# xeTaiz/vit-tf

Hardware: AMD Instinct MI355X
Metric: slices/sec (ViT-S/8, 512^3 vol: feature volume + 16-query similarity) (higher is better)
Workload: dtype fp16; 1 GPU; 512^3 CT-like synthetic volume (seed 0), ViT-S/8, fos 64: 1536 slices of 512x512 (N=4097) per step + 16-query similarity -> the metric's configuration (BASELINE configs[2]); engine_batch=512, weights=seeded synthetic vits8 (seed 0), parallelism=single GPU

## Files before the change

vit-tf_amd/csrc/engine.hip:

```cpp
#include "vittf_internal.h"

#include <stdlib.h>
#include <vector>

namespace {
struct ProfRec { hipEvent_t a, b; int cls; };
unsigned g_prof_mask = 0;
std::vector<ProfRec> g_prof_recs;
std::vector<hipEvent_t> g_prof_pool;

hipEvent_t prof_event() {
  if (!g_prof_pool.empty()) { hipEvent_t e = g_prof_pool.back(); g_prof_pool.pop_back(); return e; }
  hipEvent_t e;
  (void)hipEventCreate(&e);
  return e;
}

struct WsLayout {
  size_t x, h, qkv, o, fp8, fp8_bytes, tile_ctr, total;
};

WsLayout ws_layout(int d, int64_t rows, size_t fp8_bytes = 0) {
  const int64_t rp = (rows + 127) / 128 * 128;
  WsLayout l;
// ... 85 lines not shown
  if (((uintptr_t)ws & 255) != 0) return VITTF_ERR_INVALID_ARG;
  char* base = (char*)ws;
  float* X = (float*)(base + lay.x);
  void* H = base + lay.h;
  void* QKV = base + lay.qkv;
  void* O = base + lay.o;
  void* G = QKV;

  int rc;
  { ProfScope ps(VITTF_KERNEL_PATCH_EMBED, stream); rc = vittf_patch_embed_reg(cfg, w, pos, view, slice0, batch, reg_rows, n_reg, X, stream); }
  if (rc) return rc;
  const size_t esz = 2;
  const bool res_ln = !(cfg->flags & VITTF_CFG_SEPARATE_LN) && (d == 384 || d == 768);
  const int pre = (cfg->flags & VITTF_CFG_UNSCALED_Q) ? 0 : 1;
  const bool fp8_rows = !(cfg->flags & VITTF_CFG_FP8_HEAD_SCALES) && cfg->attention_fp8 && pre && d >= 768 && d % 256 == 0;
  const bool tail = d == 384 && w->tail_packed && res_ln;
  const bool qkv_as = d == 384 && w->qkv_packed && !cfg->attention_fp8;
  for (int l = 0; l < L; ++l) {
    const char* qkv_w = (const char*)w->qkv_w + (size_t)l * 3 * d * d * esz;
    if (res_ln ? l == 0 : true) {
      ProfScope ps(VITTF_KERNEL_LAYERNORM, stream);
      rc = vittf_layernorm(X, w->ln1_g + (size_t)l * d, w->ln1_b + (size_t)l * d, H, rows, d, cfg->ln_eps, dt, stream);
      if (rc) return rc;
    }
    if (l == L - 1 && (part_mask & 7)) {
      ProfScope ps(VITTF_KERNEL_GEMM, stream);
      rc = vittf_gemm_kfeat_parts_reg(H, qkv_w, w->qkv_b + (size_t)l * 3 * d, rows, d, d, tokens, n_reg, part_mask & 7, q_out,
                                      k_out, v_out, dt, stream);
      if (rc || !want_t) return rc;
    }
    const float* next_g = l == L - 1 ? norm_g : w->ln1_g + (size_t)(l + 1) * d;
    const float* next_b = l == L - 1 ? norm_b : w->ln1_b + (size_t)(l + 1) * d;
    { ProfScope ps(VITTF_KERNEL_GEMM_QKV, stream);
      if (fp8_rows)
        rc = vittf_gemm_qkv_fp8(H, qkv_w, w->qkv_b + (size_t)l * 3 * d, QKV, rows, 3 * d, d, tokens, cfg->heads, dt,
                                base + lay.fp8, lay.fp8_bytes, stream);
      else if (qkv_as)
        rc = vittf_gemm_as(H, (const char*)w->qkv_packed + (size_t)l * 3 * d * d * esz, w->qkv_b + (size_t)l * 3 * d, QKV, rows, 3 * d, d,
                           pre ? VITTF_EPI_BIAS_QKV : VITTF_EPI_BIAS, dt, base + lay.tile_ctr, stream);
      else
        rc = vittf_gemm(H, qkv_w, w->qkv_b + (size_t)l * 3 * d, QKV, rows, 3 * d, d,
                        pre ? VITTF_EPI_BIAS_QKV : VITTF_EPI_BIAS, 0, dt, stream);
      if (!rc && rope) rc = vittf_rope_qk(QKV, rows, tokens, 1 + n_reg, cfg->heads, rope, dt, stream); }
    if (rc) return rc;
    { ProfScope ps(VITTF_KERNEL_ATTENTION, stream);
      if (fp8_rows)
        rc = vittf_attention_fp8_rows(QKV, O, batch, tokens, cfg->heads, dt, base + lay.fp8, lay.fp8_bytes, stream);
      else if (cfg->attention_fp8 && pre)
        rc = vittf_attention_fp8(QKV, O, batch, tokens, cfg->heads, dt, base + lay.fp8, lay.fp8_bytes, stream);
      else
        rc = vittf_attention(QKV, O, batch, tokens, cfg->heads, dt, pre, stream); }
    if (rc) return rc;
    if (tail) {
      ProfScope ps(VITTF_KERNEL_MLP, stream);
      rc = vittf_block_tail(O, (const char*)w->tail_packed + (size_t)l * VITTF_TAIL_STEPS * 12288 * esz, w->proj_b + (size_t)l * d,
                            w->ln2_g + (size_t)l * d, w->ln2_b + (size_t)l * d, w->fc1_b + (size_t)l * 4 * d,
                            w->fc2_b + (size_t)l * d, X, rows, d, dt, next_g, next_b, cfg->ln_eps, H, base + lay.tile_ctr,
                            stream);
      if (rc) return rc;
      continue;
    }
    { ProfScope ps(VITTF_KERNEL_GEMM_PROJ, stream);
      if (res_ln)
        rc = vittf_gemm_residual_ln(O, (const char*)w->proj_w + (size_t)l * d * d * esz, w->proj_b + (size_t)l * d, X, rows, d,
                                    d, dt, w->ln2_g + (size_t)l * d, w->ln2_b + (size_t)l * d, cfg->ln_eps, H, stream);
      else
        rc = vittf_gemm(O, (const char*)w->proj_w + (size_t)l * d * d * esz, w->proj_b + (size_t)l * d, X, rows, d, d,
                        VITTF_EPI_BIAS_RESIDUAL, 0, dt, stream); }
    if (rc) return rc;
    if (!res_ln) {
      ProfScope ps(VITTF_KERNEL_LAYERNORM, stream);
      rc = vittf_layernorm(X, w->ln2_g + (size_t)l * d, w->ln2_b + (size_t)l * d, H, rows, d, cfg->ln_eps, dt, stream);
      if (rc) return rc;
    }
    { ProfScope ps(VITTF_KERNEL_GEMM_FC1, stream);
      rc = vittf_gemm(H, (const char*)w->fc1_w + (size_t)l * 4 * d * d * esz, w->fc1_b + (size_t)l * 4 * d, G, rows,
                      4 * d, d, VITTF_EPI_BIAS_GELU, 0, dt, stream); }
    if (rc) return rc;
    { ProfScope ps(VITTF_KERNEL_GEMM_FC2, stream);
      if (res_ln)
        rc = vittf_gemm_residual_ln(G, (const char*)w->fc2_w + (size_t)l * 4 * d * d * esz, w->fc2_b + (size_t)l * d, X, rows,
                                    d, 4 * d, dt, next_g, next_b, cfg->ln_eps, H, stream);
      else
        rc = vittf_gemm(G, (const char*)w->fc2_w + (size_t)l * 4 * d * d * esz, w->fc2_b + (size_t)l * d, X, rows, d,
                        4 * d, VITTF_EPI_BIAS_RESIDUAL, 0, dt, stream); }
    if (rc) return rc;
  }
  ProfScope ps(VITTF_KERNEL_LAYERNORM, stream);
  return vittf_token_features(X, norm_g, norm_b, t_out, batch, tokens, 1 + n_reg, d, cfg->ln_eps, stream);
}

extern "C" int vittf_vit_qkv_features_rope(const vittf_vit_config* cfg, const vittf_vit_weights* w, const vittf_pos_embed* pos,
                                           const vittf_slice_view* view, int32_t slice0, int32_t batch, int32_t part_mask,
                                           const float* reg_rows, int32_t n_reg, const vittf_rope_table* rope, uint16_t* q_out,
                                           uint16_t* k_out, uint16_t* v_out, void* ws, size_t ws_bytes, void* stream) {
  if (part_mask <= 0 || part_mask > 7) return VITTF_ERR_INVALID_ARG;
  return vittf_vit_features(cfg, w, pos, view, slice0, batch, part_mask, reg_rows, n_reg, rope, nullptr, nullptr, q_out, k_out,
                            v_out, nullptr, ws, ws_bytes, stream);
}

extern "C" int vittf_vit_qkv_features_reg(const vittf_vit_config* cfg, const vittf_vit_weights* w, const vittf_pos_embed* pos,
                                          const vittf_slice_view* view, int32_t slice0, int32_t batch, int32_t part_mask,
                                          const float* reg_rows, int32_t n_reg, uint16_t* q_out, uint16_t* k_out,
                                          uint16_t* v_out, void* ws, size_t ws_bytes, void* stream) {
  return vittf_vit_qkv_features_rope(cfg, w, pos, view, slice0, batch, part_mask, reg_rows, n_reg, nullptr, q_out, k_out, v_out, ws,
                                     ws_bytes, stream);
}

extern "C" int vittf_vit_qkv_features(const vittf_vit_config* cfg, const vittf_vit_weights* w, const vittf_pos_embed* pos,
                                      const vittf_slice_view* view, int32_t slice0, int32_t batch, int32_t part_mask,
                                      uint16_t* q_out, uint16_t* k_out, uint16_t* v_out, void* ws, size_t ws_bytes,
// ... 43 lines not shown
```

vit-tf_amd/csrc/tail_fx.hip:

```cpp
#include "vittf_common.h"

#include <type_traits>
#include <utility>

namespace {

constexpr int D = 384, HID = 4 * D, UNITS = HID / 32;
constexpr int SB = 24576, HB = SB / 2;
constexpr int PSTEPS = D / 32;
constexpr int LAG = 4;
constexpr int MSTEPS = 2 * UNITS + LAG;
constexpr int NSEQ = PSTEPS + MSTEPS;
constexpr int NSLOT = 4, AHEAD = NSLOT - 1;
constexpr int PIECES = SB / 1024 / 4;
constexpr int WAIT0 = (AHEAD - 2) * PIECES;
constexpr int NF = 4;
constexpr int PB_OFF = NSLOT * SB;
constexpr int PBH = 4608, PB = 2 * PBH;
constexpr int STG_ROW = 144;
constexpr int AF_SLOT = 1056, AF_H = 528;
constexpr int CONST_OFF = PB_OFF + 4 * PB;
constexpr int C_B1 = 0, C_B2 = HID, C_G1 = HID + D, C_E1 = HID + 2 * D,
              C_BP = HID + 3 * D, C_G2 = HID + 4 * D, C_E2 = HID + 5 * D,
              C_N = HID + 6 * D;
constexpr int NEXT_OFF = CONST_OFF + C_N * 4;
constexpr int LDS_BYTES = NEXT_OFF + 16;
static_assert(LDS_BYTES <= 160 * 1024, "LDS");
static_assert(AHEAD >= 3, "ring depth");
static_assert(32 * STG_ROW <= PBH && 4 * AF_SLOT <= PBH, "pair buffer");

typedef __attribute__((ext_vector_type(4))) unsigned u32x4_t;
typedef __attribute__((ext_vector_type(2))) unsigned u32x2_t;
typedef __attribute__((address_space(3))) const s16x8_t* lds_frag_ptr;
typedef __attribute__((address_space(3))) const f32x4_t* lds_f4_ptr;
typedef __attribute__((address_space(3))) f32x4_t* lds_w4_ptr;
typedef __attribute__((address_space(3))) u32x4_t* lds_wu4_ptr;
typedef __attribute__((address_space(3))) u32x2_t* lds_w2_ptr;
typedef __attribute__((address_space(3))) volatile unsigned* lds_u32_ptr;

struct Ring {
  i32x4_t rsrc;
  unsigned dma_dst;
  int src0;
  int g;
  int slot;
};

__device__ __forceinline__ s16x8_t ld_frag(const unsigned (&base)[4], int f) {
  return *(lds_frag_ptr)(base[f & 3] + (f >> 2) * 4096);
}

__device__ __forceinline__ void lds_dma16_keep(i32x4_t rsrc, unsigned lds_addr, int voff, int soff) {
  asm volatile("s_mov_b32 m0, %0\n\ts_nop 0\n\tbuffer_load_dwordx4 %1, %2, %3 offen lds"
               :: "s"(lds_addr), "v"(voff), "s"(rsrc), "s"(soff) : "memory");
}

struct Gelu3 { float x, p; };
__device__ __forceinline__ void gelu_a(Gelu3& s, float x) {
  s.x = x;
  asm volatile("" : "+v"(s.x));
  s.p = fmaf(-0.000524238159f, fabsf(s.x), 0.00741911121f);
  s.p = fmaf(s.p, fabsf(s.x), -0.0526018888f);
  s.p = fmaf(s.p, fabsf(s.x), -0.459225923f);
  asm volatile("" : "+v"(s.x), "+v"(s.p));
}
__device__ __forceinline__ void gelu_b(Gelu3& s) {
  s.p = fmaf(s.p, fabsf(s.x), -1.15109742f);
  s.p = __builtin_amdgcn_exp2f(fmaf(s.p, fabsf(s.x), -1.0f));
  asm volatile("" : "+v"(s.p));
}
__device__ __forceinline__ float gelu_c(const Gelu3& s) {
  float v = fmaf(-fabsf(s.x), s.p, fmaxf(s.x, 0.f));
  asm volatile("" : "+v"(v));
  return v;
}

template <int WAITN, bool LGKM = false>
__device__ __forceinline__ void x_wait() {
  static_assert(WAITN <= 63, "vmcnt");
  if constexpr (WAITN < 0) {
    if constexpr (LGKM) asm volatile("s_waitcnt lgkmcnt(0)\n\ts_barrier" ::: "memory");
    else asm volatile("s_barrier" ::: "memory");
// ... 57 lines not shown
      const int r = 8 * KH + 2 * (j / 3);
      if (j % 3 == 0) {
        gelu_a(s0, gprev[r]); gelu_a(s1, gprev[r + 1]);
      } else if (j % 3 == 1) {
        gelu_b(s0); gelu_b(s1);
      } else {
        const float v0 = gelu_c(s0), v1 = gelu_c(s1);
        pk[j / 3] = pack2_h16<DT>(v0, v1);
      }
    }
    __builtin_amdgcn_sched_barrier(0);
  }
  ring_advance(st);
}

template <int DT, int OH, bool LAST>
__device__ __forceinline__ void x_step(Ring& st, unsigned (&base)[4], s16x8_t (&wf)[NF], f32x16_t (&xacc)[D / 32],
                                       s16x8_t (&gf)[2], unsigned gf_addr) {
  x_wait<WAIT0>();
  const int g_next = ring_next(st), slot_free = ring_free(st);
  if constexpr (OH == 0) {
    gf[0] = *(lds_frag_ptr)(gf_addr);
    gf[1] = *(lds_frag_ptr)(gf_addr + 1024);
  }
#pragma unroll
  for (int j = 0; j < 12; ++j) {
    xacc[6 * OH + (j >> 1)] = mfma32<DT>(wf[j % NF], gf[j & 1], xacc[6 * OH + (j >> 1)]);
    ring_gap<LAST, true>(st, base, wf, j, g_next, slot_free);
    __builtin_amdgcn_sched_barrier(0);
  }
  ring_advance(st);
}

template <int DT, int WAITN, bool FIRST, bool LAST>
__device__ __forceinline__ void p_step(Ring& st, unsigned (&base)[4], s16x8_t (&wf)[NF], f32x16_t (&xacc)[D / 32],
                                       const s16x8_t (&acur)[2], s16x8_t (&anext)[2], unsigned anext_addr0, unsigned anext_addr1) {
  if constexpr (!FIRST) x_wait<WAITN>();
  const int g_next = ring_next(st), slot_free = ring_free(st);
  if constexpr (!LAST) {
    anext[0] = *(lds_frag_ptr)(anext_addr0);
    anext[1] = *(lds_frag_ptr)(anext_addr1);
  }
#pragma unroll
  for (int j = 0; j < 24; ++j) {
    xacc[j % 12] = mfma32<DT>(wf[j % NF], acur[j / 12], xacc[j % 12]);
    ring_gap<LAST, true, 24>(st, base, wf, j, g_next, slot_free);
    __builtin_amdgcn_sched_barrier(0);
  }
  ring_advance(st);
}

__device__ __forceinline__ constexpr int af_off(int s) { return (((s >> 2) & 1) ? 0 : PBH) + (s & 3) * AF_SLOT; }

struct Ctx {
  const unsigned short* abuf; const unsigned short* wpk; float* x; unsigned short* hout; unsigned* tile_ctr;
  int64_t rows; float ln_eps; int ntiles; int tile; unsigned lds0;
};
__device__ __forceinline__ unsigned uni(unsigned v) { return __builtin_amdgcn_readfirstlane(v); }
template <typename T> __device__ __forceinline__ T* uni_ptr(T* p) {
  const uint64_t v = reinterpret_cast<uint64_t>(p);
  return reinterpret_cast<T*>(((uint64_t)uni((unsigned)(v >> 32)) << 32) | uni((unsigned)v));
}
#define FX_ROLE_ENV                                                                                                       \
  const unsigned short* const abuf = uni_ptr(c.abuf);                                                                     \
  float* const x = uni_ptr(c.x);                                                                                          \
  unsigned short* const hout = uni_ptr(c.hout);                                                                           \
  unsigned* const tile_ctr = uni_ptr(c.tile_ctr);                                                                         \
  const int64_t rows = (int64_t)(((uint64_t)uni((unsigned)((uint64_t)c.rows >> 32)) << 32) | uni((unsigned)c.rows));     \
  const float ln_eps = __uint_as_float(uni(__float_as_uint(c.ln_eps)));                                                   \
  const int ntiles = (int)uni((unsigned)c.ntiles);                                                                        \
  int tile = (int)uni((unsigned)c.tile);                                                                                  \
  const unsigned lds0 = uni(c.lds0);                                                                                      \
  const int tid = threadIdx.x;                                                                                            \
  const int lane = tid & 63, wave = __builtin_amdgcn_readfirstlane(tid >> 6);                                             \
  const int rb = wave & 3;                                                                                                \
  const int h = lane >> 5, l31 = lane & 31;                                                                               \
  unsigned cl = lds0 + CONST_OFF + 16 * h;                                                                                \
  asm volatile("" : "+v"(cl));                                                                                            \
  auto cst4 = [&](int i) { return *(lds_f4_ptr)(cl + 4 * i); };             \
  const unsigned nxt = lds0 + NEXT_OFF;                                                                                   \
  Ring st;                                                                                                                \
  st.rsrc = lds_dma_rsrc(uni_ptr(c.wpk), (unsigned)(NSEQ * SB));                                                          \
  st.src0 = rb * (PIECES * 1024);                                                                                         \
  st.dma_dst = lds0;                                                                                                      \
  st.g = 0;                                                                                                               \
  st.slot = 0;                                                                                                            \
  const int aoff0 = tile_off(l31, h);                                                                                     \
  const unsigned pbuf = lds0 + PB_OFF + rb * PB;                           \
   \
  auto tile_rsrc = [&](const void* p, int64_t tile, int row_bytes) {                                                      \
    const int64_t first = tile * 128, left = rows - first;                                                                \
    const int nrows = tile < 0 || left <= 0 || !p ? 0 : left < 128 ? (int)left : 128;                                     \
    return __builtin_amdgcn_make_buffer_rsrc(const_cast<char*>(reinterpret_cast<const char*>(p)) + (nrows ? first : 0) * row_bytes, 0, \
                                             nrows * row_bytes, 0x00020000);                                              \
  };                                                                                                                      \
  (void)abuf; (void)x; (void)hout; (void)tile_ctr; (void)ln_eps; (void)ntiles; (void)l31; (void)aoff0; (void)nxt; (void)cst4; (void)tile_rsrc

template <int DT>
__device__ __attribute__((noinline)) void run_f(Ctx c) {
  FX_ROLE_ENV;
  asm volatile("s_setprio 3");
  unsigned pbl = pbuf + lane * 16;
  asm volatile("" : "+v"(pbl));
  u32x4_t fb[48];
  const int q8 = lane >> 3, c8 = lane & 7;
  __amdgpu_buffer_rsrc_t ra, rx;
  const int ao = (rb * 32 + q8) * (D * 2) + c8 * 16, xo = (rb * 32 + q8) * (D * 4) + c8 * 16;
  auto load_a = [&](int cg) {
#pragma unroll
    for (int i = 0; i < 4; ++i) fb[4 * cg + i] = __builtin_amdgcn_raw_buffer_load_b128(ra, ao + cg * 128, i * 8 * (D * 2), 0);
  };
  auto load_chunk = [&](int c) {
    const int r0 = c < 6 ? 24 + 4 * c : 4 * (c - 6);
#pragma unroll
    for (int i = 0; i < 4; ++i) fb[r0 + i] = __builtin_amdgcn_raw_buffer_load_b128(rx, xo + c * 128, i * 8 * (D * 4), 0);
  };
  const unsigned af_wr = pbuf + (c8 >> 1) * AF_SLOT + (c8 & 1) * AF_H + q8 * 16;
  auto put_a = [&](int cg) {
#pragma unroll
    for (int i = 0; i < 4; ++i) *(lds_wu4_ptr)(af_wr + af_off(4 * cg) + i * 128) = fb[4 * cg + i];
  };
  const unsigned ch_wr = pbuf + q8 * STG_ROW + c8 * 16;
  auto put_chunk = [&](int c) {
    const int r0 = c < 6 ? 24 + 4 * c : 4 * (c - 6);
#pragma unroll
    for (int i = 0; i < 4; ++i) *(lds_wu4_ptr)(ch_wr + (c & 1) * PBH + i * 8 * STG_ROW) = fb[r0 + i];
  };
  auto fetch_rows = [&](int t) {
    ra = tile_rsrc(abuf, t, D * 2);
    rx = tile_rsrc(x, t, D * 4);
#pragma unroll
    for (int cg = 0; cg < 6; ++cg) load_a(cg);
#pragma unroll
    for (int c = 0; c < 6; ++c) load_chunk(c);
    put_a(0);
  };
  fetch_rows(tile);
  asm volatile("s_waitcnt vmcnt(0)" ::: "memory");
  __syncthreads();
  while (true) {
    unsigned next_v = 0;
    if (tid == 256) next_v = atomicAdd(tile_ctr, 1u);
    unsigned base[4];
    s16x8_t hf[D / 16];
    s16x8_t wf[NF];
    f32x16_t bias_c;
    auto load_bias = [&](int at) {
#pragma unroll
      for (int q = 0; q < 4; ++q) {
// ... 35 lines not shown
    for (int f = 0; f < NF; ++f) wf[f] = ld_frag(base, f);
#pragma unroll
    for (int j = 0; j < 12; ++j) {
      ga = mfma32<DT>(wf[j % NF], hf[j], j == 0 ? bias_c : ga);
      ring_gap<false, false>(st, base, wf, j, 0, 0);
      __builtin_amdgcn_sched_barrier(0);
    }
    ring_advance(st);
    f_step<DT, 1, false, false, false>(st, base, wf, hf, ga, bias_c, gb, pk1);
    for (int u = 1; u < UNITS - 1; u += 2) {
      load_bias(C_B1 + 32 * u);
      f_step<DT, 0, true, false, true>(st, base, wf, hf, gb, bias_c, ga, pk0);
      f_step<DT, 1, true, false, false>(st, base, wf, hf, gb, bias_c, ga, pk1);
      put_gf(0);
      load_bias(C_B1 + 32 * (u + 1));
      f_step<DT, 0, true, false, true>(st, base, wf, hf, ga, bias_c, gb, pk0);
      f_step<DT, 1, true, false, false>(st, base, wf, hf, ga, bias_c, gb, pk1);
      put_gf(1);
    }
    load_bias(C_B1 + 32 * (UNITS - 1));
    f_step<DT, 0, true, false, true>(st, base, wf, hf, gb, bias_c, ga, pk0);
    f_step<DT, 1, true, true, false>(st, base, wf, hf, gb, bias_c, ga, pk1);
    put_gf(0);
    sync_wait<true>();
    ring_advance(st);
#pragma unroll
    for (int r = 0; r < 16; r += 2) {
      const float v0 = gelu_poly(gb[r]), v1 = gelu_poly(gb[r + 1]);
      const unsigned w = pack2_h16<DT>(v0, v1);
      if (r < 8) pk0[r >> 1] = w; else pk1[(r - 8) >> 1] = w;
    }
    put_gf(1);
    sync_wait<true>(); ring_advance(st);
    sync_wait(); ring_advance(st);
    sync_wait(); ring_advance(st);
    if (tid == 256) *(lds_u32_ptr)nxt = next_v;
    asm volatile("s_waitcnt vmcnt(0) lgkmcnt(0)\n\ts_barrier" ::: "memory");
    const int next = __builtin_amdgcn_readfirstlane((int)*(lds_u32_ptr)nxt);
    if (next >= ntiles) break;
    tile = next;
    fetch_rows(tile);
  }
}

template <int DT>
__device__ __attribute__((noinline)) void run_x(Ctx c) {
  FX_ROLE_ENV;
  unsigned base[4];
  asm volatile("s_waitcnt vmcnt(0)" ::: "memory");
  __syncthreads();
  s16x8_t wf[NF];
  f32x16_t xacc[D / 32];
  while (true) {
    int ln = lane;
    asm volatile("" : "+v"(ln));
    {
#pragma unroll
      for (int ot = 0; ot < D / 32; ++ot)
#pragma unroll
        for (int q = 0; q < 4; ++q) {
          const f32x4_t bv = cst4(C_BP + 32 * ot + 8 * q);
          xacc[ot][4 * q + 0] = bv[0]; xacc[ot][4 * q + 1] = bv[1]; xacc[ot][4 * q + 2] = bv[2]; xacc[ot][4 * q + 3] = bv[3];
        }
#pragma unroll
      for (int i = 0; i < 4; ++i) base[i] = lds0 + st.slot * SB + (aoff0 ^ (32 * i));
      const unsigned af_rd = pbuf + (ln >> 5) * AF_H + (ln & 31) * 16;
      s16x8_t aa[2], ab[2];
      x_wait<-1, true>();
#pragma unroll
      for (int f = 0; f < NF; ++f) wf[f] = ld_frag(base, f);
      aa[0] = *(lds_frag_ptr)(af_rd + af_off(0));
      aa[1] = *(lds_frag_ptr)(af_rd + af_off(1));
      p_step<DT, -1, true, false>(st, base, wf, xacc, aa, ab, af_rd + af_off(2), af_rd + af_off(3));
      p_step<DT, -1, false, false>(st, base, wf, xacc, ab, aa, af_rd + af_off(4), af_rd + af_off(5));
#pragma unroll
      for (int p = 2; p < PSTEPS - 2; p += 2) {
        p_step<DT, WAIT0, false, false>(st, base, wf, xacc, aa, ab, af_rd + af_off(2 * p + 2), af_rd + af_off(2 * p + 3));
        p_step<DT, WAIT0, false, false>(st, base, wf, xacc, ab, aa, af_rd + af_off(2 * p + 4), af_rd + af_off(2 * p + 5));
      }
      p_step<DT, WAIT0, false, false>(st, base, wf, xacc, aa, ab, af_rd + af_off(2 * PSTEPS - 2), af_rd + af_off(2 * PSTEPS - 1));
      p_step<DT, WAIT0, false, true>(st, base, wf, xacc, ab, aa, 0, 0);
      const unsigned ch_rd = pbuf + (ln & 31) * STG_ROW + 16 * (ln >> 5);
#pragma unroll
      for (int r = 0; r < 12; ++r) {
        sync_wait<true>();
        f32x4_t xv[4];
#pragma unroll
        for (int g = 0; g < 4; ++g) xv[g] = *(lds_f4_ptr)(ch_rd + (r & 1) * PBH + 32 * g);
#pragma unroll
        for (int g = 0; g < 4; ++g)
#pragma unroll
          for (int e = 0; e < 4; ++e) xacc[r][4 * g + e] += xv[g][e];
      }
      float s = 0.f;
#pragma unroll
      for (int ot = 0; ot < D / 32; ++ot) {
#pragma unroll
        for (int g = 0; g < 4; ++g) s += (xacc[ot][4 * g + 0] + xacc[ot][4 * g + 1]) + (xacc[ot][4 * g + 2] + xacc[ot][4 * g + 3]);
        __builtin_amdgcn_sched_barrier(0);
      }
      {
        const auto sw = __builtin_amdgcn_permlane32_swap(__float_as_uint(s), __float_as_uint(s), false, false);
        s = __uint_as_float(sw[0]) + __uint_as_float(sw[1]);
      }
      const float mean = s / (float)D;
      float q = 0.f;
#pragma unroll
      for (int ot = 0; ot < D / 32; ++ot) {
#pragma unroll
        for (int r = 0; r < 16; ++r) { const float dv = xacc[ot][r] - mean; q += dv * dv; }
        __builtin_amdgcn_sched_barrier(0);
      }
      {
        const auto sw = __builtin_amdgcn_permlane32_swap(__float_as_uint(q), __float_as_uint(q), false, false);
        q = __uint_as_float(sw[0]) + __uint_as_float(sw[1]);
      }
      const float rstd = 1.0f / sqrtf(q / (float)D + ln_eps);
      float mean_p = mean;
      asm volatile("" : "+v"(mean_p));
      const unsigned hw_ = pbuf + ln * 16;
      f32x4_t gq[2][4], bq[2][4];
#pragma unroll
      for (int g = 0; g < 4; ++g) { gq[0][g] = cst4(C_G2 + 8 * g); bq[0][g] = cst4(C_E2 + 8 * g); }
#pragma unroll
      for (int ot = 0; ot < D / 32; ++ot) {
        if (ot + 1 < D / 32) {
#pragma unroll
          for (int g = 0; g < 4; ++g) { gq[(ot + 1) & 1][g] = cst4(C_G2 + 32 * (ot + 1) + 8 * g); bq[(ot + 1) & 1][g] = cst4(C_E2 + 32 * (ot + 1) + 8 * g); }
        }
#pragma unroll
        for (int k2 = 0; k2 < 2; ++k2) {
          u32x4_t pk;
#pragma unroll
          for (int g2_ = 0; g2_ < 2; ++g2_) {
            const int g = 2 * k2 + g2_;
            const f32x4_t gg = gq[ot & 1][g], bb = bq[ot & 1][g];
            pk[2 * g2_ + 0] = pack2_h16<DT>((xacc[ot][4 * g + 0] - mean_p) * rstd * gg[0] + bb[0], (xacc[ot][4 * g + 1] - mean_p) * rstd * gg[1] + bb[1]);
            pk[2 * g2_ + 1] = pack2_h16<DT>((xacc[ot][4 * g + 2] - mean_p) * rstd * gg[2] + bb[2], (xacc[ot][4 * g + 3] - mean_p) * rstd * gg[3] + bb[3]);
          }
          *(lds_wu4_ptr)(hw_ + (ot & 1) * PBH + k2 * 1024) = pk;
        }
        sync_wait<true>();
      }
    }
    s16x8_t gf[2];
    x_idle_step<WAIT0>(st); x_idle_step<WAIT0>(st); x_idle_step<WAIT0>(st);
    x_wait<WAIT0>();
    {
      const int g_next = ring_next(st), slot_free = ring_free(st);
#pragma unroll
      for (int i = 0; i < PIECES; ++i) ring_piece(st, i, g_next, slot_free);
      ring_advance(st);
#pragma unroll
      for (int i = 0; i < 4; ++i) base[i] = lds0 + st.slot * SB + HB + (aoff0 ^ (32 * i));
#pragma unroll
      for (int f = 0; f < NF; ++f) wf[f] = ld_frag(base, f);
    }
    const unsigned gfa = pbuf + ln * 16;
    for (int u = 0; u < UNITS - 2; u += 2) {
      x_step<DT, 0, false>(st, base, wf, xacc, gf, gfa);
      x_step<DT, 1, false>(st, base, wf, xacc, gf, gfa);
      x_step<DT, 0, false>(st, base, wf, xacc, gf, gfa + PBH);
      x_step<DT, 1, false>(st, base, wf, xacc, gf, gfa + PBH);
    }
    x_step<DT, 0, false>(st, base, wf, xacc, gf, gfa);
    x_step<DT, 1, false>(st, base, wf, xacc, gf, gfa);
    x_step<DT, 0, false>(st, base, wf, xacc, gf, gfa + PBH);
    x_step<DT, 1, true>(st, base, wf, xacc, gf, gfa + PBH);
    asm volatile("s_waitcnt vmcnt(0) lgkmcnt(0)\n\ts_barrier" ::: "memory");
    const int next = __builtin_amdgcn_readfirstlane((int)*(lds_u32_ptr)nxt);
    {
      const auto rxo = tile_rsrc(x, tile, D * 4);
      const auto rho = tile_rsrc(hout, tile, D * 2);
      int le = lane;
      asm volatile("" : "+v"(le));
      const unsigned stg_wr_e = pbuf + (le & 31) * STG_ROW + 16 * (le >> 5);
      const unsigned stg_wh = pbuf + (le & 31) * STG_ROW + 8 * (le >> 5);
      const unsigned stg_rd_e = pbuf + (le >> 3) * STG_ROW + (le & 7) * 16;
      const int xo_e = (rb * 32 + (le >> 3)) * (D * 4) + (le & 7) * 16;
      const int ho = (rb * 32 + (le >> 3)) * (D * 2) + (le & 7) * 16;
      float s = 0.f;
      {
        f32x4_t bvq[2][4];
#pragma unroll
        for (int g = 0; g < 4; ++g) bvq[0][g] = cst4(C_B2 + 8 * g);
#pragma unroll
        for (int ot = 0; ot < D / 32; ++ot) {
#pragma unroll
          for (int g = 0; g < 4; ++g) {
            const f32x4_t bv = bvq[ot & 1][g];
            f32x4_t v;
            v[0] = xacc[ot][4 * g + 0] + bv[0]; v[1] = xacc[ot][4 * g + 1] + bv[1];
            v[2] = xacc[ot][4 * g + 2] + bv[2]; v[3] = xacc[ot][4 * g + 3] + bv[3];
#pragma unroll
            for (int e = 0; e < 4; ++e) xacc[ot][4 * g + e] = v[e];
            *(lds_w4_ptr)(stg_wr_e + 32 * g) = v;
            s += (v[0] + v[1]) + (v[2] + v[3]);
          }
          __builtin_amdgcn_sched_barrier(0);
          f32x4_t rbk[4];
#pragma unroll
          for (int i = 0; i < 4; ++i) rbk[i] = *(lds_f4_ptr)(stg_rd_e + i * 8 * STG_ROW);
          if (ot + 1 < D / 32) {
#pragma unroll
            for (int g = 0; g < 4; ++g) bvq[(ot + 1) & 1][g] = cst4(C_B2 + 32 * (ot + 1) + 8 * g);
          }
          __builtin_amdgcn_sched_barrier(0);
#pragma unroll
          for (int i = 0; i < 4; ++i)
            __builtin_amdgcn_raw_buffer_store_b128(__builtin_bit_cast(u32x4_t, rbk[i]), rxo, xo_e + ot * 128, i * 8 * (D * 4), 0);
          __builtin_amdgcn_sched_barrier(0);
        }
      }
      if (hout) {
        {
          const auto sw = __builtin_amdgcn_permlane32_swap(__float_as_uint(s), __float_as_uint(s), false, false);
          s = __uint_as_float(sw[0]) + __uint_as_float(sw[1]);
        }
        const float mean = s / (float)D;
        float q = 0.f;
#pragma unroll
        for (int ot = 0; ot < D / 32; ++ot) {
#pragma unroll
          for (int r = 0; r < 16; ++r) { const float dv = xacc[ot][r] - mean; q += dv * dv; }
          __builtin_amdgcn_sched_barrier(0);
        }
        {
          const auto sw = __builtin_amdgcn_permlane32_swap(__float_as_uint(q), __float_as_uint(q), false, false);
          q = __uint_as_float(sw[0]) + __uint_as_float(sw[1]);
        }
        const float rstd = 1.0f / sqrtf(q / (float)D + ln_eps);
        float mean_p = mean;
        asm volatile("" : "+v"(mean_p));
        f32x4_t gq1[2][4], bq1[2][4];
#pragma unroll
        for (int g = 0; g < 4; ++g) { gq1[0][g] = cst4(C_G1 + 8 * g); bq1[0][g] = cst4(C_E1 + 8 * g); }
#pragma unroll
        for (int ot = 0; ot < D / 32; ++ot) {
          const int op = ot >> 1, o2 = ot & 1;
#pragma unroll
          for (int g = 0; g < 4; ++g) {
            const f32x4_t gg = gq1[ot & 1][g], bb = bq1[ot & 1][g];
            u32x2_t pk;
            pk[0] = pack2_h16<DT>((xacc[ot][4 * g + 0] - mean_p) * rstd * gg[0] + bb[0], (xacc[ot][4 * g + 1] - mean_p) * rstd * gg[1] + bb[1]);
            pk[1] = pack2_h16<DT>((xacc[ot][4 * g + 2] - mean_p) * rstd * gg[2] + bb[2], (xacc[ot][4 * g + 3] - mean_p) * rstd * gg[3] + bb[3]);
            *(lds_w2_ptr)(stg_wh + 64 * o2 + 16 * g) = pk;
          }
          __builtin_amdgcn_sched_barrier(0);
          [[maybe_unused]] f32x4_t rbk[4];
          if (o2) {
#pragma unroll
            for (int i = 0; i < 4; ++i) rbk[i] = *(lds_f4_ptr)(stg_rd_e + i * 8 * STG_ROW);
          }
          if (ot + 1 < D / 32) {
#pragma unroll
            for (int g = 0; g < 4; ++g) { gq1[(ot + 1) & 1][g] = cst4(C_G1 + 32 * (ot + 1) + 8 * g); bq1[(ot + 1) & 1][g] = cst4(C_E1 + 32 * (ot + 1) + 8 * g); }
          }
          __builtin_amdgcn_sched_barrier(0);
          if (o2) {
#pragma unroll
            for (int i = 0; i < 4; ++i)
              __builtin_amdgcn_raw_buffer_store_b128(__builtin_bit_cast(u32x4_t, rbk[i]), rho, ho + op * 128, i * 8 * (D * 2), 0);
            __builtin_amdgcn_sched_barrier(0);
          }
        }
      }
    }
    if (next >= ntiles) break;
    tile = next;
  }
}

template <int DT>
__global__ __launch_bounds__(512, 1) void tail_fx_kernel(const unsigned short* __restrict__ abuf, const unsigned short* __restrict__ wpk,
                                                         const float* __restrict__ bp, const float* __restrict__ g2, const float* __restrict__ e2,
                                                         const float* __restrict__ b1, const float* __restrict__ b2,
                                                         float* __restrict__ x, int64_t rows, const float* __restrict__ ln_g,
                                                         const float* __restrict__ ln_b, float ln_eps,
                                                         unsigned short* __restrict__ hout, int ntiles,
                                                         unsigned* __restrict__ tile_ctr) {
  __shared__ __attribute__((aligned(16))) char smem[LDS_BYTES];
  const int tid = threadIdx.x;
  const int lane = tid & 63, wave = __builtin_amdgcn_readfirstlane(tid >> 6);
  float* const cst = reinterpret_cast<float*>(smem + CONST_OFF);
  for (int i = tid; i < C_N; i += 512) {
    float v;
    if (i < C_B2) v = b1[i];
    else if (i < C_G1) v = b2[i - C_B2];
    else if (i < C_E1) v = ln_g ? ln_g[i - C_G1] : 1.f;
    else if (i < C_BP) v = ln_b ? ln_b[i - C_E1] : 0.f;
    else if (i < C_G2) v = bp[i - C_BP];
    else if (i < C_E2) v = g2[i - C_G2];
    else v = e2[i - C_E2];
    cst[i] = v;
  }
  const unsigned lds0 = (unsigned)(size_t)LDS_PTR(smem);
  const unsigned nxt = lds0 + NEXT_OFF;
  if (tid == 0) *(lds_u32_ptr)nxt = atomicAdd(tile_ctr, 1u);
  __syncthreads();
  const int tile = __builtin_amdgcn_readfirstlane((int)*(lds_u32_ptr)nxt);
  if (tile >= ntiles) return;
  if (wave < 4) {
    const i32x4_t rsrc = lds_dma_rsrc(wpk, (unsigned)(NSEQ * SB));
#pragma unroll
    for (int u = 0; u < AHEAD; ++u)
#pragma unroll
      for (int i = 0; i < PIECES; ++i)
        lds_dma16(rsrc, lds0 + wave * (PIECES * 1024) + u * SB + i * 1024, lane * 16, u * SB + wave * (PIECES * 1024) + i * 1024);
  }
  const Ctx c = {abuf, wpk, x, hout, tile_ctr, rows, ln_eps, ntiles, tile, lds0};
  if (wave >= 4) run_f<DT>(c);
  else run_x<DT>(c);
  asm volatile("s_waitcnt vmcnt(0)" ::: "memory");
}

}

extern "C" size_t vittf_block_tail_workspace_bytes(void) { return sizeof(unsigned); }

extern "C" int vittf_block_tail(const void* attn_out, const void* w_packed, const float* proj_b, const float* ln2_g,
                                const float* ln2_b, const float* b1, const float* b2, float* x, int64_t rows, int32_t d,
                                int32_t dtype, const float* ln_g, const float* ln_b, float ln_eps, void* h_out, void* tile_counter,
                                void* stream) {
  if (!attn_out || !w_packed || !proj_b || !ln2_g || !ln2_b || !b1 || !b2 || !x || rows <= 0) return VITTF_ERR_INVALID_ARG;
  if (d != D) return VITTF_ERR_INVALID_ARG;
  if ((ln_g || ln_b || h_out) && !(ln_g && ln_b && h_out)) return VITTF_ERR_INVALID_ARG;
  const int64_t tiles = (rows + 127) / 128;
  if (tiles > 0x7fffffff) return VITTF_ERR_INVALID_ARG;
  if ((((uintptr_t)attn_out | (uintptr_t)w_packed | (uintptr_t)x | (uintptr_t)h_out) & 15) != 0) return VITTF_ERR_INVALID_ARG;
  if (!tile_counter || ((uintptr_t)tile_counter & 3) != 0) return VITTF_ERR_INVALID_ARG;
  const int cus = vittf_current_cus();
  if (cus <= 0) return VITTF_ERR_NO_DEVICE;
  const unsigned grid = (unsigned)(tiles < cus ? tiles : cus);
  hipStream_t st = (hipStream_t)stream;
  unsigned* ctr = (unsigned*)tile_counter;
  if (hipMemsetAsync(ctr, 0, sizeof(unsigned), st) != hipSuccess) return VITTF_ERR_LAUNCH;
#define FX_LAUNCH(DTV)                                                                                               \
  hipLaunchKernelGGL((tail_fx_kernel<DTV>), dim3(grid), dim3(512), 0, st, (const unsigned short*)attn_out,           \
                     (const unsigned short*)w_packed, proj_b, ln2_g, ln2_b, b1, b2, x, rows, ln_g, ln_b, ln_eps,     \
                     (unsigned short*)h_out, (int)tiles, ctr)
  if (dtype == VITTF_BF16) FX_LAUNCH(VITTF_BF16);
  else if (dtype == VITTF_FP16) FX_LAUNCH(VITTF_FP16);
  else return VITTF_ERR_INVALID_ARG;
#undef FX_LAUNCH
  vittf_note_kernel(VITTF_KERNEL_MLP, "tail_fx_kernel");
  return vittf_check_launch();
}
```

vit-tf_amd/csrc/vittf_internal.h:

```cpp
#pragma once
#include "vittf_common.h"

static inline size_t align256(size_t x) { return (x + 255) & ~(size_t)255; }

static inline int64_t vittf_kfeat_out_bytes(int64_t rows, int32_t d, int32_t tokens, int32_t drop) {
  return (rows - rows / tokens * drop) * (int64_t)d * 2;
}

bool vittf_gemm_rows_covers(int32_t n, int32_t k, int64_t rows);
int vittf_gemm_rows(const void* a, const void* w, const float* bias, float* x, int64_t rows, int32_t n, int32_t k,
                    int32_t dtype, const float* ln_g, const float* ln_b, float ln_eps, void* h, hipStream_t st);

bool vittf_gemm_pp_covers(int32_t k, int32_t columns, const void* a, const void* w);
bool vittf_gemm_pp_covers_out(const void* out, int64_t kfeat_bytes);
int vittf_gemm_pp(const void* a, const void* w, const float* bias, void* out, int64_t rows, int32_t n, int32_t k,
                  int32_t epilogue, int32_t tokens, int32_t dtype, hipStream_t st);
int vittf_gemm_pp_kfeat_parts(const void* a, const void* w, const float* bias, int64_t rows, int32_t d, int32_t k,
                              int32_t tokens, int32_t n_reg, int32_t part_mask, void* const outs[3], int32_t dtype,
                              hipStream_t st, int32_t* taken);

void vittf_fp8_ws_pointers(void* ws, int32_t batch, int32_t tokens, int32_t heads, unsigned** amax, unsigned char** q8,
                           unsigned char** k8, unsigned char** qs, unsigned char** ks, int32_t* np);

int vittf_attention_pp64(const void* qkv, void* out, int32_t batch, int32_t tokens, int32_t heads, int32_t dtype,
                         hipStream_t st);

size_t vittf_sim_mfma_workspace_bytes(int32_t classes, int32_t annotations);
bool vittf_sim_mfma_applies(int32_t f, int32_t classes, int32_t total_a, const void* ws, size_t ws_bytes, const void* feat,
                            int64_t nvox);
int vittf_sim_mfma_maps(const unsigned short* feat, int32_t f, int64_t nvox, const float* qf, const int32_t* class_start_host,
                        int32_t classes, const float* voxel_norm, float* sim, unsigned* maxbits, void* ws, size_t ws_bytes,
                        hipStream_t st);
```

Baseline: 2282 slices/s.

## Skip residual store in penultimate tail and double-buffer epilogue LDS staging

Adds a store_x flag to the fused block-tail kernel so the penultimate layer, when only key features are wanted, skips writing the fp32 residual stream back to global memory. The epilogue staging now alternates between the pair buffer and an idle ring slot, so writes for the next column block can proceed before the previous block's read-back and global store finish, and H stores are deferred by one iteration. Lane indices are recomputed via mbcnt to cut live registers. This relies on the last ring slot being unused at drain time; if the final X is needed elsewhere, skipping the store could break correctness.

```diff
diff --git a/vit-tf_amd/csrc/engine.hip b/vit-tf_amd/csrc/engine.hip
--- a/vit-tf_amd/csrc/engine.hip
+++ b/vit-tf_amd/csrc/engine.hip
@@ -161,11 +161,12 @@
         rc = vittf_attention(QKV, O, batch, tokens, cfg->heads, dt, pre, stream); }
     if (rc) return rc;
     if (tail) {
+      const int store_x = !(l == L - 2 && (part_mask & 7) && !want_t);
       ProfScope ps(VITTF_KERNEL_MLP, stream);
-      rc = vittf_block_tail(O, (const char*)w->tail_packed + (size_t)l * VITTF_TAIL_STEPS * 12288 * esz, w->proj_b + (size_t)l * d,
+      rc = vittf_block_tail_opt(O, (const char*)w->tail_packed + (size_t)l * VITTF_TAIL_STEPS * 12288 * esz, w->proj_b + (size_t)l * d,
                             w->ln2_g + (size_t)l * d, w->ln2_b + (size_t)l * d, w->fc1_b + (size_t)l * 4 * d,
                             w->fc2_b + (size_t)l * d, X, rows, d, dt, next_g, next_b, cfg->ln_eps, H, base + lay.tile_ctr,
-                            stream);
+                            store_x, (hipStream_t)stream);
       if (rc) return rc;
       continue;
     }
diff --git a/vit-tf_amd/csrc/tail_fx.hip b/vit-tf_amd/csrc/tail_fx.hip
--- a/vit-tf_amd/csrc/tail_fx.hip
+++ b/vit-tf_amd/csrc/tail_fx.hip
@@ -1,4 +1,4 @@
-#include "vittf_common.h"
+#include "vittf_internal.h"
 
 #include <type_traits>
 #include <utility>
@@ -28,6 +28,9 @@
 static_assert(LDS_BYTES <= 160 * 1024, "LDS");
 static_assert(AHEAD >= 3, "ring depth");
 static_assert(32 * STG_ROW <= PBH && 4 * AF_SLOT <= PBH, "pair buffer");
+constexpr int STG2 = SB / 4;
+static_assert(NSEQ % NSLOT == 0, "every row tile starts at ring slot 0: the last slot is idle from the drain to the next step 0");
+static_assert(32 * STG_ROW <= STG2 && STG2 == PIECES * 1024, "second staging buffer inside the wave's own pieces of the slot");
 
 typedef __attribute__((ext_vector_type(4))) unsigned u32x4_t;
 typedef __attribute__((ext_vector_type(2))) unsigned u32x2_t;
@@ -191,9 +194,15 @@
 
 __device__ __forceinline__ constexpr int af_off(int s) { return (((s >> 2) & 1) ? 0 : PBH) + (s & 3) * AF_SLOT; }
 
+__device__ __forceinline__ int lane_now() {
+  int l;
+  asm volatile("v_mbcnt_lo_u32_b32 %0, -1, 0\n\tv_mbcnt_hi_u32_b32 %0, -1, %0" : "=&v"(l));
+  return l;
+}
+
 struct Ctx {
   const unsigned short* abuf; const unsigned short* wpk; float* x; unsigned short* hout; unsigned* tile_ctr;
-  int64_t rows; float ln_eps; int ntiles; int tile; unsigned lds0;
+  int64_t rows; float ln_eps; int store_x; int tile; unsigned lds0;
 };
 __device__ __forceinline__ unsigned uni(unsigned v) { return __builtin_amdgcn_readfirstlane(v); }
 template <typename T> __device__ __forceinline__ T* uni_ptr(T* p) {
@@ -207,9 +216,10 @@
   unsigned* const tile_ctr = uni_ptr(c.tile_ctr);                                                                         \
   const int64_t rows = (int64_t)(((uint64_t)uni((unsigned)((uint64_t)c.rows >> 32)) << 32) | uni((unsigned)c.rows));     \
   const float ln_eps = __uint_as_float(uni(__float_as_uint(c.ln_eps)));                                                   \
-  const int ntiles = (int)uni((unsigned)c.ntiles);                                                                        \
+  const int ntiles = (int)((rows + 127) / 128);                                     \
   int tile = (int)uni((unsigned)c.tile);                                                                                  \
   const unsigned lds0 = uni(c.lds0);                                                                                      \
+  const bool store_x = uni((unsigned)c.store_x) != 0;                   \
   const int tid = threadIdx.x;                                                                                            \
   const int lane = tid & 63, wave = __builtin_amdgcn_readfirstlane(tid >> 6);                                             \
   const int rb = wave & 3;                                                                                                \
@@ -233,7 +243,7 @@
     return __builtin_amdgcn_make_buffer_rsrc(const_cast<char*>(reinterpret_cast<const char*>(p)) + (nrows ? first : 0) * row_bytes, 0, \
                                              nrows * row_bytes, 0x00020000);                                              \
   };                                                                                                                      \
-  (void)abuf; (void)x; (void)hout; (void)tile_ctr; (void)ln_eps; (void)ntiles; (void)l31; (void)aoff0; (void)nxt; (void)cst4; (void)tile_rsrc
+  (void)abuf; (void)x; (void)hout; (void)store_x; (void)tile_ctr; (void)ln_eps; (void)ntiles; (void)l31; (void)aoff0; (void)nxt; (void)cst4; (void)tile_rsrc
 
 template <int DT>
 __device__ __attribute__((noinline)) void run_f(Ctx c) {
@@ -375,8 +385,8 @@
   s16x8_t wf[NF];
   f32x16_t xacc[D / 32];
   while (true) {
-    int ln = lane;
-    asm volatile("" : "+v"(ln));
+    const int ln = lane_now();
+    const int aoff_x = tile_off(ln & 31, ln >> 5);
     {
 #pragma unroll
       for (int ot = 0; ot < D / 32; ++ot)
@@ -386,7 +396,7 @@
           xacc[ot][4 * q + 0] = bv[0]; xacc[ot][4 * q + 1] = bv[1]; xacc[ot][4 * q + 2] = bv[2]; xacc[ot][4 * q + 3] = bv[3];
         }
 #pragma unroll
-      for (int i = 0; i < 4; ++i) base[i] = lds0 + st.slot * SB + (aoff0 ^ (32 * i));
+      for (int i = 0; i < 4; ++i) base[i] = lds0 + st.slot * SB + (aoff_x ^ (32 * i));
       const unsigned af_rd = pbuf + (ln >> 5) * AF_H + (ln & 31) * 16;
       s16x8_t aa[2], ab[2];
       x_wait<-1, true>();
@@ -475,7 +485,7 @@
       for (int i = 0; i < PIECES; ++i) ring_piece(st, i, g_next, slot_free);
       ring_advance(st);
 #pragma unroll
-      for (int i = 0; i < 4; ++i) base[i] = lds0 + st.slot * SB + HB + (aoff0 ^ (32 * i));
+      for (int i = 0; i < 4; ++i) base[i] = lds0 + st.slot * SB + HB + (aoff_x ^ (32 * i));
 #pragma unroll
       for (int f = 0; f < NF; ++f) wf[f] = ld_frag(base, f);
     }
@@ -492,46 +502,55 @@
     x_step<DT, 1, true>(st, base, wf, xacc, gf, gfa + PBH);
     asm volatile("s_waitcnt vmcnt(0) lgkmcnt(0)\n\ts_barrier" ::: "memory");
     const int next = __builtin_amdgcn_readfirstlane((int)*(lds_u32_ptr)nxt);
+    asm volatile("" :: "s"(next));
     {
-      const auto rxo = tile_rsrc(x, tile, D * 4);
+      const auto rxo = tile_rsrc(store_x ? x : nullptr, tile, D * 4);
       const auto rho = tile_rsrc(hout, tile, D * 2);
-      int le = lane;
-      asm volatile("" : "+v"(le));
+      const int le = lane_now();
       const unsigned stg_wr_e = pbuf + (le & 31) * STG_ROW + 16 * (le >> 5);
-      const unsigned stg_wh = pbuf + (le & 31) * STG_ROW + 8 * (le >> 5);
       const unsigned stg_rd_e = pbuf + (le >> 3) * STG_ROW + (le & 7) * 16;
+      const unsigned stg2 = lds0 + (NSLOT - 1) * SB + rb * STG2 - pbuf;
       const int xo_e = (rb * 32 + (le >> 3)) * (D * 4) + (le & 7) * 16;
-      const int ho = (rb * 32 + (le >> 3)) * (D * 2) + (le & 7) * 16;
       float s = 0.f;
+      f32x4_t rbk[4];
+      auto read_back = [&](unsigned rd, int round) {
+#pragma unroll
+        for (int i = 0; i < 4; ++i) rbk[i] = *(lds_f4_ptr)(rd + (round & 1) * stg2 + i * 8 * STG_ROW);
+      };
+      auto store_x_rows = [&](int ot) {
+#pragma unroll
+        for (int i = 0; i < 4; ++i)
+          __builtin_amdgcn_raw_buffer_store_b128(__builtin_bit_cast(u32x4_t, rbk[i]), rxo, xo_e + ot * 128, i * 8 * (D * 4), 0);
+      };
       {
-        f32x4_t bvq[2][4];
-#pragma unroll
-        for (int g = 0; g < 4; ++g) bvq[0][g] = cst4(C_B2 + 8 * g);
+        f32x4_t bvq[4];
+#pragma unroll
+        for (int g = 0; g < 4; ++g) bvq[g] = cst4(C_B2 + 8 * g);
 #pragma unroll
         for (int ot = 0; ot < D / 32; ++ot) {
 #pragma unroll
           for (int g = 0; g < 4; ++g) {
-            const f32x4_t bv = bvq[ot & 1][g];
+            const f32x4_t bv = bvq[g];
             f32x4_t v;
-            v[0] = xacc[ot][4 * g + 0] + bv[0]; v[1] = xacc[ot][4 * g + 1] + bv[1];
-            v[2] = xacc[ot][4 * g + 2] + bv[2]; v[3] = xacc[ot][4 * g + 3] + bv[3];
+#pragma unroll
+            for (int e = 0; e < 4; ++e) v[e] = xacc[ot][4 * g + e] + bv[e];
 #pragma unroll
             for (int e = 0; e < 4; ++e) xacc[ot][4 * g + e] = v[e];
-            *(lds_w4_ptr)(stg_wr_e + 32 * g) = v;
-            s += (v[0] + v[1]) + (v[2] + v[3]);
+            *(lds_w4_ptr)(stg_wr_e + (ot & 1) * stg2 + 32 * g) = v;
           }
           __builtin_amdgcn_sched_barrier(0);
-          f32x4_t rbk[4];
-#pragma unroll
-          for (int i = 0; i < 4; ++i) rbk[i] = *(lds_f4_ptr)(stg_rd_e + i * 8 * STG_ROW);
+          read_back(stg_rd_e, ot);
           if (ot + 1 < D / 32) {
 #pragma unroll
-            for (int g = 0; g < 4; ++g) bvq[(ot + 1) & 1][g] = cst4(C_B2 + 32 * (ot + 1) + 8 * g);
+            for (int g = 0; g < 4; ++g) bvq[g] = cst4(C_B2 + 32 * (ot + 1) + 8 * g);
           }
           __builtin_amdgcn_sched_barrier(0);
 #pragma unroll
-          for (int i = 0; i < 4; ++i)
-            __builtin_amdgcn_raw_buffer_store_b128(__builtin_bit_cast(u32x4_t, rbk[i]), rxo, xo_e + ot * 128, i * 8 * (D * 4), 0);
+          for (int g = 0; g < 4; ++g)
+            s += (xacc[ot][4 * g + 0] + xacc[ot][4 * g + 1]) + (xacc[ot][4 * g + 2] + xacc[ot][4 * g + 3]);
+          asm volatile("" : "+v"(s));
+          __builtin_amdgcn_sched_barrier(0);
+          store_x_rows(ot);
           __builtin_amdgcn_sched_barrier(0);
         }
       }
@@ -555,38 +574,42 @@
         const float rstd = 1.0f / sqrtf(q / (float)D + ln_eps);
         float mean_p = mean;
         asm volatile("" : "+v"(mean_p));
-        f32x4_t gq1[2][4], bq1[2][4];
-#pragma unroll
-        for (int g = 0; g < 4; ++g) { gq1[0][g] = cst4(C_G1 + 8 * g); bq1[0][g] = cst4(C_E1 + 8 * g); }
+        const int lh = lane_now();
+        const unsigned stg_wh = pbuf + (lh & 31) * STG_ROW + 8 * (lh >> 5);
+        const unsigned stg_rd_h = pbuf + (lh >> 3) * STG_ROW + (lh & 7) * 16;
+        const int ho = (rb * 32 + (lh >> 3)) * (D * 2) + (lh & 7) * 16;
+        auto store_h_rows = [&](int op) {
+#pragma unroll
+          for (int i = 0; i < 4; ++i)
+            __builtin_amdgcn_raw_buffer_store_b128(__builtin_bit_cast(u32x4_t, rbk[i]), rho, ho + op * 128, i * 8 * (D * 2), 0);
+        };
+        f32x4_t gq1[4], bq1[4];
+#pragma unroll
+        for (int g = 0; g < 4; ++g) { gq1[g] = cst4(C_G1 + 8 * g); bq1[g] = cst4(C_E1 + 8 * g); }
 #pragma unroll
         for (int ot = 0; ot < D / 32; ++ot) {
           const int op = ot >> 1, o2 = ot & 1;
 #pragma unroll
           for (int g = 0; g < 4; ++g) {
-            const f32x4_t gg = gq1[ot & 1][g], bb = bq1[ot & 1][g];
+            const f32x4_t gg = gq1[g], bb = bq1[g];
             u32x2_t pk;
             pk[0] = pack2_h16<DT>((xacc[ot][4 * g + 0] - mean_p) * rstd * gg[0] + bb[0], (xacc[ot][4 * g + 1] - mean_p) * rstd * gg[1] + bb[1]);
             pk[1] = pack2_h16<DT>((xacc[ot][4 * g + 2] - mean_p) * rstd * gg[2] + bb[2], (xacc[ot][4 * g + 3] - mean_p) * rstd * gg[3] + bb[3]);
-            *(lds_w2_ptr)(stg_wh + 64 * o2 + 16 * g) = pk;
+            *(lds_w2_ptr)(stg_wh + (op & 1) * stg2 + 64 * o2 + 16 * g) = pk;
           }
           __builtin_amdgcn_sched_barrier(0);
-          [[maybe_unused]] f32x4_t rbk[4];
-          if (o2) {
-#pragma unroll
-            for (int i = 0; i < 4; ++i) rbk[i] = *(lds_f4_ptr)(stg_rd_e + i * 8 * STG_ROW);
+          if (!o2 && op > 0) {
+            store_h_rows(op - 1);
+            __builtin_amdgcn_sched_barrier(0);
           }
           if (ot + 1 < D / 32) {
 #pragma unroll
-            for (int g = 0; g < 4; ++g) { gq1[(ot + 1) & 1][g] = cst4(C_G1 + 32 * (ot + 1) + 8 * g); bq1[(ot + 1) & 1][g] = cst4(C_E1 + 32 * (ot + 1) + 8 * g); }
+            for (int g = 0; g < 4; ++g) { gq1[g] = cst4(C_G1 + 32 * (ot + 1) + 8 * g); bq1[g] = cst4(C_E1 + 32 * (ot + 1) + 8 * g); }
           }
+          if (o2) read_back(stg_rd_h, op);
           __builtin_amdgcn_sched_barrier(0);
-          if (o2) {
-#pragma unroll
-            for (int i = 0; i < 4; ++i)
-              __builtin_amdgcn_raw_buffer_store_b128(__builtin_bit_cast(u32x4_t, rbk[i]), rho, ho + op * 128, i * 8 * (D * 2), 0);
-            __builtin_amdgcn_sched_barrier(0);
-          }
         }
+        store_h_rows(D / 64 - 1);
       }
     }
     if (next >= ntiles) break;
@@ -601,7 +624,7 @@
                                                          float* __restrict__ x, int64_t rows, const float* __restrict__ ln_g,
                                                          const float* __restrict__ ln_b, float ln_eps,
                                                          unsigned short* __restrict__ hout, int ntiles,
-                                                         unsigned* __restrict__ tile_ctr) {
+                                                         unsigned* __restrict__ tile_ctr, int store_x) {
   __shared__ __attribute__((aligned(16))) char smem[LDS_BYTES];
   const int tid = threadIdx.x;
   const int lane = tid & 63, wave = __builtin_amdgcn_readfirstlane(tid >> 6);
@@ -631,7 +654,7 @@
       for (int i = 0; i < PIECES; ++i)
         lds_dma16(rsrc, lds0 + wave * (PIECES * 1024) + u * SB + i * 1024, lane * 16, u * SB + wave * (PIECES * 1024) + i * 1024);
   }
-  const Ctx c = {abuf, wpk, x, hout, tile_ctr, rows, ln_eps, ntiles, tile, lds0};
+  const Ctx c = {abuf, wpk, x, hout, tile_ctr, rows, ln_eps, store_x, tile, lds0};
   if (wave >= 4) run_f<DT>(c);
   else run_x<DT>(c);
   asm volatile("s_waitcnt vmcnt(0)" ::: "memory");
@@ -641,13 +664,13 @@
 
 extern "C" size_t vittf_block_tail_workspace_bytes(void) { return sizeof(unsigned); }
 
-extern "C" int vittf_block_tail(const void* attn_out, const void* w_packed, const float* proj_b, const float* ln2_g,
-                                const float* ln2_b, const float* b1, const float* b2, float* x, int64_t rows, int32_t d,
-                                int32_t dtype, const float* ln_g, const float* ln_b, float ln_eps, void* h_out, void* tile_counter,
-                                void* stream) {
+int vittf_block_tail_opt(const void* attn_out, const void* w_packed, const float* proj_b, const float* ln2_g, const float* ln2_b,
+                         const float* b1, const float* b2, float* x, int64_t rows, int32_t d, int32_t dtype, const float* ln_g,
+                         const float* ln_b, float ln_eps, void* h_out, void* tile_counter, int32_t store_x, hipStream_t st) {
   if (!attn_out || !w_packed || !proj_b || !ln2_g || !ln2_b || !b1 || !b2 || !x || rows <= 0) return VITTF_ERR_INVALID_ARG;
   if (d != D) return VITTF_ERR_INVALID_ARG;
   if ((ln_g || ln_b || h_out) && !(ln_g && ln_b && h_out)) return VITTF_ERR_INVALID_ARG;
+  if (!store_x && !h_out) return VITTF_ERR_INVALID_ARG;
   const int64_t tiles = (rows + 127) / 128;
   if (tiles > 0x7fffffff) return VITTF_ERR_INVALID_ARG;
   if ((((uintptr_t)attn_out | (uintptr_t)w_packed | (uintptr_t)x | (uintptr_t)h_out) & 15) != 0) return VITTF_ERR_INVALID_ARG;
@@ -655,13 +678,12 @@
   const int cus = vittf_current_cus();
   if (cus <= 0) return VITTF_ERR_NO_DEVICE;
   const unsigned grid = (unsigned)(tiles < cus ? tiles : cus);
-  hipStream_t st = (hipStream_t)stream;
   unsigned* ctr = (unsigned*)tile_counter;
   if (hipMemsetAsync(ctr, 0, sizeof(unsigned), st) != hipSuccess) return VITTF_ERR_LAUNCH;
 #define FX_LAUNCH(DTV)                                                                                               \
   hipLaunchKernelGGL((tail_fx_kernel<DTV>), dim3(grid), dim3(512), 0, st, (const unsigned short*)attn_out,           \
                      (const unsigned short*)w_packed, proj_b, ln2_g, ln2_b, b1, b2, x, rows, ln_g, ln_b, ln_eps,     \
-                     (unsigned short*)h_out, (int)tiles, ctr)
+                     (unsigned short*)h_out, (int)tiles, ctr, store_x ? 1 : 0)
   if (dtype == VITTF_BF16) FX_LAUNCH(VITTF_BF16);
   else if (dtype == VITTF_FP16) FX_LAUNCH(VITTF_FP16);
   else return VITTF_ERR_INVALID_ARG;
@@ -669,3 +691,11 @@
   vittf_note_kernel(VITTF_KERNEL_MLP, "tail_fx_kernel");
   return vittf_check_launch();
 }
+
+extern "C" int vittf_block_tail(const void* attn_out, const void* w_packed, const float* proj_b, const float* ln2_g,
+                                const float* ln2_b, const float* b1, const float* b2, float* x, int64_t rows, int32_t d,
+                                int32_t dtype, const float* ln_g, const float* ln_b, float ln_eps, void* h_out, void* tile_counter,
+                                void* stream) {
+  return vittf_block_tail_opt(attn_out, w_packed, proj_b, ln2_g, ln2_b, b1, b2, x, rows, d, dtype, ln_g, ln_b, ln_eps, h_out,
+                              tile_counter, 1, (hipStream_t)stream);
+}
diff --git a/vit-tf_amd/csrc/vittf_internal.h b/vit-tf_amd/csrc/vittf_internal.h
--- a/vit-tf_amd/csrc/vittf_internal.h
+++ b/vit-tf_amd/csrc/vittf_internal.h
@@ -19,6 +19,10 @@
                               int32_t tokens, int32_t n_reg, int32_t part_mask, void* const outs[3], int32_t dtype,
                               hipStream_t st, int32_t* taken);
 
+int vittf_block_tail_opt(const void* attn_out, const void* w_packed, const float* proj_b, const float* ln2_g, const float* ln2_b,
+                         const float* b1, const float* b2, float* x, int64_t rows, int32_t d, int32_t dtype, const float* ln_g,
+                         const float* ln_b, float ln_eps, void* h_out, void* tile_counter, int32_t store_x, hipStream_t st);
+
 void vittf_fp8_ws_pointers(void* ws, int32_t batch, int32_t tokens, int32_t heads, unsigned** amax, unsigned char** q8,
                            unsigned char** k8, unsigned char** qs, unsigned char** ks, int32_t* np);
 
```

Result: no change. 2299 slices/s (median of 6 runs) (+0.8%).
